# smithlabcode/walt

Measured on AMD Instinct MI355X. Metric: mapped reads/sec (100 bp single-end, hg19-scale index, -m 6 -b 5000), higher is better.
Workload: dtype u32

## Files before the change

### walt_amd/csrc/device_common.h

```cpp
#ifndef WALT_AMD_DEVICE_COMMON_H_
#define WALT_AMD_DEVICE_COMMON_H_

#include <hip/hip_runtime.h>

#include <initializer_list>
#include <mutex>
#include <string>
#include <type_traits>
#include <vector>

#include "../../include/walt_amd.h"
#include "batch_host.h"
#include "host_common.h"
#include "index_core.h"

#define WALT_HIP(expr)                                                                       \
  do {                                                                                       \
    hipError_t e_ = (expr);                                                                  \
    if (e_ != hipSuccess)                                                                    \
      return walt::fail(WALT_EHIP, std::string(#expr) + ": " + hipGetErrorString(e_));       \
  } while (0)

#define WALT_HIP_FORKED(expr)                                                                \
  do {                                                                                       \
    hipError_t e_ = (expr);                                                                  \
    if (e_ != hipSuccess) {                                                                  \
      unwind();                                                                              \
      return walt::fail(WALT_EHIP, std::string(#expr) + ": " + hipGetErrorString(e_));       \
    }                                                                                        \
  } while (0)

struct walt_options {
  int se_pipe = 1;
  long long se_heavy_chunk = 0;
  int se_stage_blocks = 0;
  int se_verify_blocks = 0;
  int se_stagger = 0;
  int se_lit_ablate = 0;
  int se_lit_side = 1;
  int se_lit_staged = 0;
  long long se_defer_min = -1;
  int se_stage_occ = 0;
  int se_carry = 1;
  int se_heavy_mono = 0;
  long long grid = 0;
  int pe_mode = 0;
  long long pe_chunk = 0;
  long long pe_rounds = 0;
  long long pe_stage_cap = 0;
  int pe_small_heaps = 0;
  int pe_serial = 0;
  int pe_push_wide = 0;
  long long pe_defer_min = -1;
  int pe_lit_fuse = 1;
  int pe_roomy = -1;
  int pile_rows = 0;
  long long pile_extract_blocks = 0;
};

struct walt_index {
  int device = 0;
  int n_cu = 256;
  walt_options opt;
  walt::IndexHead head;
  std::vector<uint32_t> start_index;
  walt::IndexView view;
  std::vector<void*> allocs;
// ... 267 lines not shown
```

### walt_amd/csrc/device_index.hip

```cpp
#include <fcntl.h>
#include <stdio.h>
#include <stdlib.h>
#include <string.h>
#include <time.h>
#include <unistd.h>

#include <algorithm>
#include <atomic>
#include <cstring>
#include <thread>

#include <hip/hip_runtime.h>
#include <rocprim/rocprim.hpp>

#include <stddef.h>

#include "device_common.h"

namespace walt {


__global__ void k_pack_genome(const uint8_t* __restrict__ bytes, uint32_t len, uint32_t ga,
                              uint32_t* __restrict__ g2, uint32_t nwords, uint32_t* __restrict__ err) {
  uint32_t w = blockIdx.x * blockDim.x + threadIdx.x;
// ... 988 lines not shown
}
const char* walt_index_chrom_name(const walt_index* idx, uint32_t i) {
  return idx && i < idx->head.names.size() ? idx->head.names[i].c_str() : "";
}
uint64_t walt_index_genome_len(const walt_index* idx) { return idx ? idx->head.genome_len : 0; }
uint64_t walt_index_device_bytes(const walt_index* idx) { return idx ? idx->device_bytes : 0; }
int walt_index_dir_bits(const walt_index* idx) { return idx ? (int)idx->view.dir_bits : -1; }
uint64_t walt_index_bad_buckets(const walt_index* idx, int strand) {
  return idx && strand >= 0 && strand < 4 ? idx->bad_buckets[strand] : 0;
}
namespace {
struct OptionName {
  const char* name;
  int kind;
  size_t offset;
  long long lo, hi;
};
#define WALT_OPT_I(f, lo, hi) {#f, 0, offsetof(walt_options, f), lo, hi}
#define WALT_OPT_L(f, lo, hi) {#f, 1, offsetof(walt_options, f), lo, hi}
const OptionName kOptions[] = {
    WALT_OPT_I(se_pipe, 0, 1),        WALT_OPT_L(se_heavy_chunk, 0, 1ll << 28), WALT_OPT_I(se_lit_staged, 0, 1), WALT_OPT_I(se_stage_blocks, 0, 16), WALT_OPT_I(se_verify_blocks, 0, 16), WALT_OPT_I(se_stagger, 0, 1), WALT_OPT_I(se_lit_side, 0, 2), WALT_OPT_I(se_lit_ablate, 0, 7),
    WALT_OPT_L(se_defer_min, -1, 1ll << 30), WALT_OPT_I(se_stage_occ, 0, 4),   WALT_OPT_I(se_carry, 0, 1),
    WALT_OPT_I(se_heavy_mono, 0, 1),  WALT_OPT_L(grid, 0, 1ll << 20),           WALT_OPT_I(pe_mode, 0, 1),
    WALT_OPT_L(pe_chunk, 0, 1ll << 28), WALT_OPT_L(pe_rounds, 0, 4),            WALT_OPT_L(pe_stage_cap, 0, 1ll << 28),
    WALT_OPT_I(pe_small_heaps, 0, 1), WALT_OPT_I(pe_serial, 0, 1), WALT_OPT_I(pe_push_wide, 0, 1),              WALT_OPT_L(pe_defer_min, -1, 1ll << 30),
    WALT_OPT_I(pe_roomy, -1, 1),      WALT_OPT_I(pe_lit_fuse, 0, 1),
    WALT_OPT_I(pile_rows, 0, 1),      WALT_OPT_L(pile_extract_blocks, 0, 1ll << 16),
};
#undef WALT_OPT_I
#undef WALT_OPT_L
const OptionName* find_option(const char* name) {
  if (!name) return nullptr;
  for (const OptionName& o : kOptions)
    if (!strcmp(o.name, name)) return &o;
  return nullptr;
}
}

int walt_index_set_option(walt_index* idx, const char* name, long long value) {
  if (!idx) return fail(WALT_EINVAL, "null index");
  const OptionName* o = find_option(name);
  if (!o) return fail(WALT_EINVAL, std::string("walt_index_set_option: unknown option '") + (name ? name : "(null)") + "'");
  if (value < o->lo || value > o->hi)
    return fail(WALT_EINVAL, std::string("walt_index_set_option: ") + name + " = " + std::to_string(value) + " is outside [" +
                                 std::to_string(o->lo) + ", " + std::to_string(o->hi) + "]");
  char* base = reinterpret_cast<char*>(&idx->opt) + o->offset;
// ... 25 lines not shown
```

### walt_amd/csrc/map_se.hip

```cpp
#include <stdio.h>
#include <stdlib.h>
#include <string.h>

#include "map_common.h"
#include "map_items.h"

namespace walt {

static __global__ __launch_bounds__(kBlock) void k_ascii_to_2bit(const uint8_t* __restrict__ bases,
                                                                  const uint64_t* __restrict__ offsets, uint32_t n,
                                                                  uint32_t* __restrict__ codes2, uint64_t cap_bytes,
                                                                  uint32_t* __restrict__ err) {
  const uint64_t o0 = offsets[0], all = offsets[n] - o0, total = all < cap_bytes ? all : cap_bytes;
  if (all > cap_bytes && blockIdx.x == 0 && threadIdx.x == 0) atomicAdd(err + 1, 1u);
  const uint8_t* src = bases + o0;
  const uint32_t mis = (uint32_t)(reinterpret_cast<uintptr_t>(src) & 15);
  const uint64_t nwords = (total + 15) / 16;
  uint32_t bad_total = 0;
  for (uint64_t i = (uint64_t)blockIdx.x * blockDim.x + threadIdx.x; i < nwords;
       i += (uint64_t)gridDim.x * blockDim.x) {
    uint32_t qs[4] = {0, 0, 0, 0};
    const uint64_t b0 = 16 * i;
    if (mis == 0 && b0 + 16 <= total) {
      const uint4 q = *reinterpret_cast<const uint4*>(src + b0);
      qs[0] = q.x; qs[1] = q.y; qs[2] = q.z; qs[3] = q.w;
    } else {
      for (uint64_t k = b0; k < b0 + 16; ++k) {
        const uint32_t c = k < total ? src[k] : 0x41u;
// ... 1369 lines not shown
  ItemQueue q;
  q.items = hs.items; q.ctl = hs.ctl; q.cap = 2 * hs.hcap; q.ovf = err + 2;
  q.bigs = hs.giants; q.big_n = hs.ctl + 5; q.big_cap = hs.hcap / 8;
  if (DENSE && blockIdx.x == 0 && threadIdx.x == 0) items_overflow_check(q);
  uint32_t n_big = DENSE ? *q.big_n : 0u;
  n_big = n_big < q.big_cap ? n_big : q.big_cap;
  const uint32_t n_items = q.ctl[DENSE ? 0 : 1] + n_big;
  if (n_items == 0) return;
  __shared__ uint32_t s_start[kLdsChroms + 1];
  __shared__ uint32_t s_edge[DENSE ? kEdgeWords : 1];
  const bool fits = iv.n_chrom <= kLdsChroms;
  chrom_tab_stage(s_start, iv.start_index, chrom_tab_of(iv.n_chrom));
  if (DENSE && iv.edge_bits != nullptr)
    for (uint32_t i = threadIdx.x; i < kEdgeWords; i += blockDim.x) s_edge[i] = iv.edge_bits[i];
  __syncthreads();
  const uint32_t* const edge = (DENSE && iv.edge_bits != nullptr) ? s_edge : nullptr;
  SummarySink sink;
  sink.sums = hs.sums; sink.hcap = hs.hcap; sink.n_verified = 0; sink.b = b; sink.tail = 0; sink.in_region = 0;
  if (fits) item_stream<NW, DENSE, true, SummarySink, G>(iv, strand_base, q, n_items, s_start, sink, n_big, edge);
  else item_stream<NW, DENSE, false, SummarySink, G>(iv, strand_base, q, n_items, s_start, sink, n_big, edge);
  flush_counters({0u, sink.n_verified, 0u}, 0u, stats);
}

#ifndef WALT_LIT_OCC
#define WALT_LIT_OCC 5
#endif
template <int NW, bool LITERAL = true>
__global__ __launch_bounds__(kBlock, NW <= 8 ? WALT_LIT_OCC : 1) void k_map_se_literal(IndexView iv, const uint32_t* __restrict__ codes2,
                                                            const uint64_t* __restrict__ offsets,
                                                            uint32_t* __restrict__ err, uint32_t strand_base,
                                                            uint32_t max_mm,
                                                            uint32_t b, const uint32_t* __restrict__ mask_table,
                                                            BestMatch* __restrict__ out,
                                                            unsigned long long* __restrict__ stats,
                                                            uint32_t* __restrict__ defer_count,
                                                            uint32_t* __restrict__ defer_list,
                                                            uint32_t all_reads, const uint32_t* __restrict__ range = nullptr) {
  uint32_t n_entries = 0;
  if (range != nullptr) {
    const uint32_t lo_entry = range[0];
    n_entries = range[1] > lo_entry ? range[1] - lo_entry : 0u;
    if (n_entries == 0) return;
    defer_list += lo_entry;
  }
  __shared__ BlockShared sh;
  const uint32_t* si = block_prologue(sh, iv, mask_table, strand_base);
// ... 39 lines not shown
}
static SeGeometry se_geometry_for(uint32_t n, int nw, bool pipe, uint64_t chunk_hook) {
  SeGeometry g;
  const uint64_t share = ((uint64_t)n + (pipe ? 7 : 3)) / (pipe ? 8 : 4);
  g.hcap = (uint32_t)align_up(n <= 65536 ? (n ? n : 1) : (share > 65536 ? share : 65536), 64);
  if (chunk_hook > 0 && chunk_hook * 8 >= n) g.hcap = (uint32_t)align_up(chunk_hook, 64);
  const uint32_t k = (uint32_t)(((uint64_t)n + g.hcap - 1) / g.hcap);
  g.piped = pipe && k > 1;
  g.chunks = g.piped ? (k + 1u) & ~1u : k;
  g.slot_bytes = se_heavy_slot_bytes(g.hcap, nw);
  g.heavy_bytes = 16 + kHeavyCtlWords * 4 + (g.piped ? 2 : 1) * g.slot_bytes;
  return g;
}
static uint64_t se_heavy_bytes(uint32_t n, int nw) {
  const uint64_t a = se_geometry_for(n, nw, true, 0).heavy_bytes, c = se_geometry_for(n, nw, false, 0).heavy_bytes;
  return a > c ? a : c;
}
static SeGeometry se_geometry(uint32_t n, int nw, const walt_options& opt) {
  SeGeometry g = se_geometry_for(n, nw, opt.se_pipe != 0, opt.se_heavy_chunk > 0 ? (uint64_t)opt.se_heavy_chunk : 0);
  if (g.heavy_bytes > se_heavy_bytes(n, nw) || g.hcap > (1u << kStageJBits)) g = se_geometry_for(n, nw, opt.se_pipe != 0, 0);
  return g;
}
static uint64_t se_carry_bytes(uint32_t n) { return (uint64_t)kPat * se_stride(n) * 16; }

constexpr unsigned kLiteralGrid = 2048;

#if defined(WALT_DIAG)
static uint32_t g_ablate = 0;
static unsigned long long* g_stamps = nullptr;
static void debug_sync(const char* what, hipStream_t stream) {
  static const bool on = getenv("WALT_AMD_SYNC_DEBUG") != nullptr;
  if (!on) return;
  const hipError_t e = hipStreamSynchronize(stream);
  fprintf(stderr, "[walt_amd sync] %s: %s\n", what, hipGetErrorString(e));
}
#else
static void debug_sync(const char*, hipStream_t) {}
#endif

unsigned persistent_grid(const walt_index* idx) {
  return idx->opt.grid > 0 ? (unsigned)idx->opt.grid : (unsigned)idx->n_cu * 8u;
}

template <int NW>
static int launch_map_se(walt_index* idx, const IndexView& view, const uint32_t* codes2, const uint64_t* offsets, uint32_t* err,
                         uint32_t n, uint32_t strand_base, uint32_t max_mm, uint32_t b, BestMatch* out,
                         unsigned long long* stats, uint32_t* defer_count, uint32_t* defer_list, uint64_t stride,
                         uint32_t* heavy_area, uint4* carry_area, hipStream_t stream) {
  const walt_options& opt = idx->opt;
  const unsigned pg = persistent_grid(idx);
  const unsigned g1 = grid_for(n) < pg ? grid_for(n) : pg;
  uint32_t* heavy_count = defer_count + 24;
  uint32_t* heavy_list = defer_list + 2 * stride;
  const bool mono = opt.se_heavy_mono != 0;
  SeCarry carry;
  carry.st = (opt.se_carry && !mono) ? carry_area : nullptr;
  carry.neg = carry_area + stride;
  carry.stride = stride;
  idx->n_detail = 0;
  auto mark = [&](unsigned char kind) {
    if (!idx->profile || idx->n_detail >= walt_index::kDetailEvents) return;
    hipEvent_t& e = idx->ev_detail[idx->n_detail];
    if (!e && hipEventCreate(&e) != hipSuccess) return;
    if (hipEventRecord(e, stream) != hipSuccess) return;
    idx->ev_kind[idx->n_detail++] = kind;
  };
  mark(255);
#if defined(WALT_DIAG)
  const bool diag = g_ablate != 0 || g_stamps != nullptr;
  const char* sm = getenv("WALT_AMD_STAMPS");
  const int stamp_mode = sm ? atoi(sm) : 0;
// ... 21 lines not shown
  };
  uint32_t* const rng = heavy_area + kHeavyCtlWords - 8;
  if (mono) {
#if defined(WALT_DIAG)
    if (diag2)
      hipLaunchKernelGGL((k_map_se<NW, true, true>), dim3(g1), dim3(kBlock), 0, stream, view, codes2, offsets, err, n,
                         strand_base, max_mm, b, idx->d_mask_table, out, stats, defer_count, defer_list, heavy_count,
                         heavy_list, g_ablate, g_stamps, SeCarry());
    else
#endif
      hipLaunchKernelGGL((k_map_se<NW, false, true>), dim3(g1), dim3(kBlock), 0, stream, view, codes2, offsets, err, n,
                         strand_base, max_mm, b, idx->d_mask_table, out, stats, defer_count, defer_list, heavy_count,
                         heavy_list, 0u, nullptr, SeCarry());
  } else {
    const SeGeometry geo = se_geometry(n, NW, opt);
    const uint32_t hcap = geo.hcap;
    const bool piped = geo.piped && !diag;
    const uint32_t chunks = geo.chunks;
    HeavyStage hs;
    hs.ctl = heavy_area;
    hs.hcap = hcap;
    hs.even = piped ? 1u : 0u;
    const uint64_t slot_words = geo.slot_bytes / 4;
    auto use_slot = [&](uint32_t k, uint32_t*& lists) {
      lists = heavy_area + kHeavyCtlWords + k * slot_words;
      hs.st = reinterpret_cast<uint4*>(lists + (uint64_t)kPat * hcap);
      hs.rdq = hs.st + hcap;
      hs.sums = hs.rdq + (uint64_t)rd_quads<NW>() * hcap;
      hs.items = hs.sums + (uint64_t)(kPat + 1) * hcap;
      hs.giants = hs.items + (uint64_t)2 * hcap * item_quads<NW>();
    };
    hs.defer_min = opt.se_defer_min < 0 ? (uint32_t)kSmallRegion
                 : opt.se_defer_min == 0 ? 0xFFFFFFFFu
                 : (uint32_t)(opt.se_defer_min < (long long)kSmallRegion ? (long long)kSmallRegion : opt.se_defer_min);
    hs.lit_ablate = (uint32_t)opt.se_lit_ablate;
    uint32_t* const ctl0 = heavy_area;
    static const int vb_dense = [] {
      int nb = 0;
      if (hipOccupancyMaxActiveBlocksPerMultiprocessor(&nb, k_se_verify<NW, NW <= 10>, kBlock, 0) != hipSuccess || nb < 1) nb = 4;
      return nb;
    }();
    static const int vb_gather = [] {
      int nb = 0;
      if (hipOccupancyMaxActiveBlocksPerMultiprocessor(&nb, k_se_verify<NW, false>, kBlock, 0) != hipSuccess || nb < 1) nb = 2;
      return nb;
    }();
    const unsigned vg_dense = (unsigned)vb_dense * (unsigned)idx->n_cu, vg_gather = (unsigned)vb_gather * (unsigned)idx->n_cu;
    const bool lit_staged = opt.se_lit_staged != 0 && !diag;
    lit_side = !lit_staged && opt.se_lit_side != 0 && !diag && n <= kDeferMask;
    uint32_t* const ctl2 = ctl0 + 64 * kPat;
    uint32_t* const rng_side = ctl2 + 32;
    static_assert(8 * kPat * kLitChunks >= 34, "the side launch's control words fit the literal rounds' area");
    if (lit_side && !idx->se_side) {
      int lo_pri = 0, hi_pri = 0;
      WALT_HIP(hipDeviceGetStreamPriorityRange(&lo_pri, &hi_pri));
      WALT_HIP(create_stream_set(&idx->se_side, &lo_pri, {&idx->se_fork, &idx->se_join}));
    }
    if (piped && !idx->se_pipe)
      WALT_HIP(create_stream_set(&idx->se_pipe, nullptr, {&idx->se_pipe_ev[0], &idx->se_pipe_ev[1], &idx->se_pipe_ev[2]}));
    const bool lit_early = lit_side && opt.se_lit_side >= 2;
    if (lit_early) {
      hipLaunchKernelGGL(k_lit_snapshot, dim3(1), dim3(64), 0, stream, defer_count, ctl2, rng_side);
      WALT_HIP(hipEventRecord(idx->se_fork, stream));
      WALT_HIP(hipStreamWaitEvent(idx->se_side, idx->se_fork, 0));
      forked = true;
      launch_bin_deferred(ctl2, defer_list, defer_list + stride, idx->se_side);
      const unsigned g_lit = grid_for(n) < kLiteralGrid ? grid_for(n) : kLiteralGrid;
      hipLaunchKernelGGL(k_map_se_literal<NW>, dim3(g_lit), dim3(kBlock), 0, idx->se_side, view, codes2, offsets, err,
                         strand_base, max_mm, b, idx->d_mask_table, out, stats, ctl2, defer_list + stride, 0u);
// ... 39 lines not shown
            WALT_HIP_FORKED(hipEventRecord(idx->se_fork, cs));
            WALT_HIP_FORKED(hipStreamWaitEvent(idx->se_side, idx->se_fork, 0));
            launch_bin_deferred(ctl3, defer_list, defer_list + stride, idx->se_side, ctl3 + 1);
            const unsigned g_lit = grid_for(n) < kLiteralGrid ? grid_for(n) : kLiteralGrid;
            hipLaunchKernelGGL(k_map_se_literal<NW>, dim3(g_lit), dim3(kBlock), 0, idx->se_side, view, codes2, offsets, err,
                               strand_base, max_mm, b, idx->d_mask_table, out, stats, defer_count, defer_list + stride, 0u, ctl3 + 24);
            WALT_HIP_FORKED(hipEventRecord(idx->se_join, idx->se_side));
          }
          if (lit_side && !lit_early && c_side == (piped ? 1u : 0u)) {
            if (piped) WALT_HIP_FORKED(hipStreamWaitEvent(cs, idx->se_pipe_ev[1], 0));
            hipLaunchKernelGGL(k_lit_snapshot, dim3(1), dim3(64), 0, cs, defer_count, ctl2, rng_side);
            WALT_HIP_FORKED(hipEventRecord(idx->se_fork, cs));
            WALT_HIP_FORKED(hipStreamWaitEvent(idx->se_side, idx->se_fork, 0));
            forked = true;
            launch_bin_deferred(ctl2, defer_list, defer_list + stride, idx->se_side);
            const unsigned g_lit = grid_for(n) < kLiteralGrid ? grid_for(n) : kLiteralGrid;
            hipLaunchKernelGGL(k_map_se_literal<NW>, dim3(g_lit), dim3(kBlock), 0, idx->se_side, view, codes2, offsets, err,
                               strand_base, max_mm, b, idx->d_mask_table, out, stats, ctl2, defer_list + stride, 0u);
            WALT_HIP_FORKED(hipEventRecord(idx->se_join, idx->se_side));
          }
        }
        if constexpr (NW <= 10 && long_seed_nw<NW>())
          hipLaunchKernelGGL((k_se_tail_narrow<NW>), dim3(pg), dim3(kBlock), 0, cs, view, strand_base, hs, b);
        if constexpr (NW <= 10) {
          hipLaunchKernelGGL((k_se_verify<NW, true>), dim3(vgd), dim3(kBlock), 0, cs, view, strand_base, stats, hs, b, err);
        }
        hipLaunchKernelGGL((k_se_verify<NW, false>), dim3(vg_gather), dim3(kBlock), 0, cs, view, strand_base, stats, hs, b, err);
        if (marks) mark(lit ? 3 : 2);
      }
      return WALT_OK;
    };
    for (uint32_t c = 0; c < chunks; ++c) {
      const bool odd = piped && (c & 1u);
      forked = forked || odd;
      uint32_t* lists = nullptr;
      use_slot(odd ? 1u : 0u, lists);
      hs.first = c * hcap;
      hs.chunk = c;
      if (piped && lit_side && !lit_early && c == 2) WALT_HIP_FORKED(hipStreamWaitEvent(stream, idx->se_fork, 0));
      const int rc_chunk = run_chunk(odd ? idx->se_pipe : stream, ctl0 + 8 * kPat * c, lists, false, heavy_count, heavy_list, carry, !odd, c);
      if (rc_chunk) return rc_chunk;
    }
    if (piped) {
      WALT_HIP_FORKED(hipEventRecord(idx->se_pipe_ev[2], idx->se_pipe));
      WALT_HIP_FORKED(hipStreamWaitEvent(stream, idx->se_pipe_ev[2], 0));
    }
    if (lit_staged) {
      hs.even = 0;
// ... 51 lines not shown
    WALT_HIP(hipMemset(g_stamps, 0, 16 * sizeof(unsigned long long)));
  }
  return WALT_OK;
}
#endif

static int se_check_len(uint32_t max_read_len, int& nw) {
  nw = nw_for_len(max_read_len);
  if (!nw) return fail(WALT_EINVAL, "read length above 1024 is not supported (reference line limit is 1000, util.hpp:43)");
  if (max_read_len > kMaxReadLen)
    return fail(WALT_EINVAL, "reads longer than " + std::to_string(kMaxReadLen) + " bases are outside the tables of seed pattern " +
                                 std::to_string(kPat) + " (seedpattern.hpp)");
  return WALT_OK;
}

struct SeWorkspace {
  uint32_t* err;
  unsigned long long* shards;
  uint32_t* defer_count;
  uint32_t* defer_list;
  uint32_t* codes2;
  uint32_t* heavy_area;
  uint4* carry_area;
  uint64_t stride;
  uint64_t end;
};
static SeWorkspace se_workspace(void* d_workspace, uint32_t n, uint32_t max_read_len, int nw) {
  SeWorkspace w;
  w.stride = se_stride(n);
  w.err = reinterpret_cast<uint32_t*>(d_workspace);
  w.shards = reinterpret_cast<unsigned long long*>(w.err + 64);
  w.defer_count = w.err + 32;
  w.defer_list = w.err + 64 + kStatShardBytes / 4;
  w.codes2 = w.defer_list + 3 * w.stride;
  w.heavy_area = reinterpret_cast<uint32_t*>(
      align_up(reinterpret_cast<uint64_t>(w.codes2 + codes2_words((uint64_t)n * max_read_len)), 16));
  w.carry_area = reinterpret_cast<uint4*>(align_up(reinterpret_cast<uint64_t>(w.heavy_area) + se_heavy_bytes(n, nw), 16));
  w.end = reinterpret_cast<uint64_t>(w.carry_area) + se_carry_bytes(n);
  return w;
}

static int se_map_pass(walt_index* idx, const IndexView& view, const SeWorkspace& w, const uint64_t* offsets, uint32_t n,
                       int nw, uint32_t sb, uint32_t max_mm, uint32_t b, BestMatch* out, hipStream_t stream) {
  return dispatch_nw(nw, [&](auto NW) {
    return launch_map_se<decltype(NW)::value>(idx, view, w.codes2, offsets, w.err, n, sb, max_mm, b, out, w.shards, w.defer_count,
                                              w.defer_list, w.stride, w.heavy_area, w.carry_area, stream);
  });
}

struct SeCall {
  std::unique_lock<std::mutex> busy;
  int nw = 0;
  SeWorkspace w;
  IndexView view;
  const uint64_t* offsets = nullptr;
};
static int se_begin(walt_index* idx, bool rp, bool locked, const void* d_bases, const void* d_offsets, uint32_t n,
                    uint32_t max_read_len, void* d_workspace, size_t workspace_bytes, hipStream_t stream, SeCall& c) {
  const std::string entry = rp ? "walt_map_se_rpbat_batch" : "walt_map_se_batch";
  if (n > kDeferMask + 1) return fail(WALT_EINVAL, "more than 2^28 reads in one batch (the reference's -N limit is 10^8, walt.cpp:236-239)");
  if (!locked)
    if (const int rc_busy = take_busy(c.busy, idx->se_busy, entry.c_str(), "single-end")) return rc_busy;
#if defined(WALT_DIAG)
  if (const int rc_diag = se_diag_setup()) return rc_diag;
#endif
  if (const int rc_len = se_check_len(max_read_len, c.nw)) return rc_len;
  const size_t need = rp ? walt_se_rpbat_workspace_bytes(n, max_read_len) : walt_se_workspace_bytes(n, max_read_len);
  if (workspace_bytes < need)
    return fail(WALT_EINVAL, entry + "_device: the workspace holds " + std::to_string(workspace_bytes) + " bytes, the call needs " +
                                 std::to_string(need) + (rp ? " (walt_se_rpbat_workspace_bytes)" : " (walt_se_workspace_bytes)"));
  WALT_HIP(hipSetDevice(idx->device));
  c.w = se_workspace(d_workspace, n, max_read_len, c.nw);
  WALT_HIP(hipMemsetAsync(c.w.err, 0, 64 * sizeof(uint32_t) + kStatShardBytes, stream));
  WALT_HIP(hipMemsetAsync(c.w.heavy_area, 0, kHeavyCtlWords * sizeof(uint32_t), stream));
  c.offsets = reinterpret_cast<const uint64_t*>(d_offsets);
  if (idx->profile) WALT_HIP(hipEventRecord(idx->ev[0], stream));
  c.view = idx->view;
  c.view.batch_max_len = max_read_len;
  c.view.batch_cap_bytes = (uint64_t)n * max_read_len;
  launch_ascii_to_2bit(reinterpret_cast<const uint8_t*>(d_bases), c.offsets, n, c.w.codes2, c.view.batch_cap_bytes, c.w.err, stream);
  if (idx->profile) WALT_HIP(hipEventRecord(idx->ev[1], stream));
  return WALT_OK;
}

int map_se_device(walt_index* idx, const void* d_bases, const void* d_offsets, uint32_t n, uint32_t max_read_len,
                  int ag, uint32_t max_mm, uint32_t b, void* d_out, void* d_stats, void* d_workspace,
                  size_t workspace_bytes, hipStream_t stream, bool locked) {
  if (!idx) return fail(WALT_EINVAL, "null index");
  const unsigned need = ag ? WALT_STRANDS_GA : WALT_STRANDS_CT;
  if ((idx->strand_mask & need) != need)
    return fail(WALT_EINVAL, ag ? "index opened without the _GA10/_GA11 strands" : "index opened without the _CT00/_CT01 strands");
  if (n == 0) return WALT_OK;
  SeCall c;
  if (const int rc = se_begin(idx, false, locked, d_bases, d_offsets, n, max_read_len, d_workspace, workspace_bytes, stream, c)) return rc;
  const int rc = se_map_pass(idx, c.view, c.w, c.offsets, n, c.nw, ag ? 2u : 0u, max_mm, b, reinterpret_cast<BestMatch*>(d_out), stream);
  if (rc) return rc;
  launch_reduce_stats(c.w.shards, reinterpret_cast<unsigned long long*>(d_stats), stream);
// ... 41 lines not shown
    return fail(WALT_EINVAL, "walt_map_se_rpbat_batch: the index was opened without the strands " + missing +
                                 " (random PBAT maps under both conversions: open it with WALT_STRANDS_ALL)");
  }
  if (n == 0) return WALT_OK;
  if (!d_out || !d_conv || !d_stats || !d_workspace || (reinterpret_cast<uintptr_t>(d_out) & 15) ||
      (reinterpret_cast<uintptr_t>(d_workspace) & 15))
    return fail(WALT_EINVAL, "walt_map_se_rpbat_batch_device: bad argument (null pointer, or d_out / d_workspace not 16-byte aligned)");
  SeCall c;
  int rc = se_begin(idx, true, locked, d_bases, d_offsets, n, max_read_len, d_workspace, workspace_bytes, stream, c);
  if (rc) return rc;
  const SeWorkspace& w = c.w;
  uint4* const ga = reinterpret_cast<uint4*>(reinterpret_cast<uint8_t*>(d_workspace) + se_rpbat_ga_offset(n, max_read_len));
  unsigned long long* stats = reinterpret_cast<unsigned long long*>(d_stats);
  rc = se_map_pass(idx, c.view, w, c.offsets, n, c.nw, 0u, max_mm, b, reinterpret_cast<BestMatch*>(d_out), stream);
  if (rc) return rc;
  auto unwind = [&]() {
    if (idx->se_pipe) (void)hipStreamSynchronize(idx->se_pipe);
    if (idx->se_side) (void)hipStreamSynchronize(idx->se_side);
  };
  launch_reduce_stats(w.shards, stats, stream);
  WALT_HIP_FORKED(hipGetLastError());
  WALT_HIP_FORKED(hipMemsetAsync(w.err + 3, 0, 61 * sizeof(uint32_t), stream));
  WALT_HIP_FORKED(hipMemsetAsync(w.heavy_area, 0, kHeavyCtlWords * sizeof(uint32_t), stream));
  rc = se_map_pass(idx, c.view, w, c.offsets, n, c.nw, 2u, max_mm, b, reinterpret_cast<BestMatch*>(ga), stream);
  if (rc) {
    unwind();
    return rc;
  }
  const unsigned gm = grid_for(n) < (unsigned)idx->n_cu * 4u ? grid_for(n) : (unsigned)idx->n_cu * 4u;
  hipLaunchKernelGGL(k_se_rpbat_merge, dim3(gm), dim3(kBlock), 0, stream, reinterpret_cast<uint4*>(d_out), ga,
                     reinterpret_cast<uint8_t*>(d_conv), n);
  hipLaunchKernelGGL(k_reduce_stats<1>, dim3(1), dim3(kStatShards), 0, stream, w.shards, stats);
  if (idx->profile) {
    WALT_HIP_FORKED(hipEventRecord(idx->ev[2], stream));
    idx->ev_valid = true;
  }
  WALT_HIP_FORKED(hipGetLastError());
  return WALT_OK;
}

int check_read_errors(const void* d_workspace, hipStream_t stream) {
  uint32_t herr[3] = {0, 0, 0};
  WALT_HIP(hipMemcpyAsync(herr, d_workspace, sizeof(herr), hipMemcpyDeviceToHost, stream));
  WALT_HIP(hipStreamSynchronize(stream));
  if (herr[2]) return fail(WALT_EHIP, "internal: a work-item queue of the heavy pass overflowed (" + std::to_string(herr[2]) + " items dropped); results are incomplete");
  if (herr[1]) return fail(WALT_EINVAL, "reads longer than max_read_len, or more bases than n x max_read_len (" + std::to_string(herr[1]) + " refusals)");
// ... 61 lines not shown
  for (int i = 1; i < idx->n_detail; ++i) {
    float ms = 0.f;
    WALT_HIP(hipEventElapsedTime(&ms, idx->ev_detail[i - 1], idx->ev_detail[i]));
    if (idx->ev_kind[i] < 4) out4[idx->ev_kind[i]] += ms;
  }
  return WALT_OK;
}

int walt_profile_last(walt_index* idx, float* pack_ms, float* map_ms) {
  if (!idx || !idx->profile || !idx->ev_valid) return fail(WALT_EINVAL, "no profiled call recorded");
  WALT_HIP(hipEventSynchronize(idx->ev[2]));
  float a = 0, b = 0;
  WALT_HIP(hipEventElapsedTime(&a, idx->ev[0], idx->ev[1]));
  WALT_HIP(hipEventElapsedTime(&b, idx->ev[1], idx->ev[2]));
  if (pack_ms) *pack_ms = a;
  if (map_ms) *map_ms = b;
  return WALT_OK;
}

size_t walt_se_workspace_bytes(uint32_t n, uint32_t max_read_len) {
  int nw = nw_for_len(max_read_len);
  if (!nw) nw = 64;
  return 64 * sizeof(uint32_t) + kStatShardBytes + 3 * se_stride(n) * sizeof(uint32_t) +
         codes2_words((uint64_t)n * max_read_len) * sizeof(uint32_t) + 16 + se_heavy_bytes(n, nw) + 16 + se_carry_bytes(n);
}

int walt_map_se_batch_device(walt_index* idx, const void* d_bases, const void* d_offsets, uint32_t n,
                             uint32_t max_read_len, int ag_wildcard, uint32_t max_mismatches, uint32_t b,
                             void* d_out, void* d_stats, void* d_workspace, size_t workspace_bytes, void* stream) {
  return map_se_device(idx, d_bases, d_offsets, n, max_read_len, ag_wildcard, max_mismatches, b, d_out, d_stats,
                       d_workspace, workspace_bytes, reinterpret_cast<hipStream_t>(stream), false);
}

static int se_host_call(walt_index* idx, const char* bases, const uint64_t* offsets, uint32_t n, int ag, uint32_t max_mm,
                        uint32_t b, walt_best_match* out, uint8_t* conv, bool rp, walt_batch_stats* stats) {
  const std::string entry = rp ? "walt_map_se_rpbat_batch" : "walt_map_se_batch";
  if (!idx || !offsets || (!bases && n && offsets[n] > 0) || (!out && n) || (rp && !conv && n)) return fail(WALT_EINVAL, entry + ": bad argument");
  if (stats) memset(stats, 0, sizeof(*stats));
  if (n == 0) return WALT_OK;
  uint32_t max_len = 0;
  if (const char* bad = scan_offsets(offsets, n, &max_len)) return fail(WALT_EINVAL, bad);
  std::unique_lock<std::mutex> busy;
  if (const int rc_busy = take_busy(busy, idx->se_busy, entry.c_str(), "single-end")) return rc_busy;
  WALT_HIP(hipSetDevice(idx->device));
  const size_t ws_bytes = rp ? walt_se_rpbat_workspace_bytes(n, max_len) : walt_se_workspace_bytes(n, max_len);
  HostUpload up{idx};
  void *d_bases = nullptr, *d_off = nullptr;
// ... 39 lines not shown
```

Baseline: 1.348 billion.

## Group heavy verify items sharing a candidate range so one wavefront verifies several reads

Adds a hash-bucket sort (count, scan, scatter) of dense-verify items keyed by strand and record start. A wavefront-level cut pass then packs items with identical candidate ranges into units of up to four reads. A new shared verify kernel loads each genome window once and checks it against every read in the unit, replacing the per-item dense verify by default. This removes redundant window loads, at the cost of extra sort and cut kernels, more workspace, an added memset and more register pressure from per-read accumulators.

Result: faster. 1.458 billion (median of 6 runs) (+8.2%).

```diff
diff --git a/walt_amd/csrc/device_common.h b/walt_amd/csrc/device_common.h
--- a/walt_amd/csrc/device_common.h
+++ b/walt_amd/csrc/device_common.h
@@ -43,6 +43,9 @@
   int se_stage_occ = 0;
   int se_carry = 1;
   int se_heavy_mono = 0;
+  int se_verify_share = 1;
+  int se_share_r = 0;
+  long long se_share_cap = 0;
   long long grid = 0;
   int pe_mode = 0;
   long long pe_chunk = 0;
diff --git a/walt_amd/csrc/device_index.hip b/walt_amd/csrc/device_index.hip
--- a/walt_amd/csrc/device_index.hip
+++ b/walt_amd/csrc/device_index.hip
@@ -1034,6 +1034,7 @@
     WALT_OPT_I(se_pipe, 0, 1),        WALT_OPT_L(se_heavy_chunk, 0, 1ll << 28), WALT_OPT_I(se_lit_staged, 0, 1), WALT_OPT_I(se_stage_blocks, 0, 16), WALT_OPT_I(se_verify_blocks, 0, 16), WALT_OPT_I(se_stagger, 0, 1), WALT_OPT_I(se_lit_side, 0, 2), WALT_OPT_I(se_lit_ablate, 0, 7),
     WALT_OPT_L(se_defer_min, -1, 1ll << 30), WALT_OPT_I(se_stage_occ, 0, 4),   WALT_OPT_I(se_carry, 0, 1),
     WALT_OPT_I(se_heavy_mono, 0, 1),  WALT_OPT_L(grid, 0, 1ll << 20),           WALT_OPT_I(pe_mode, 0, 1),
+    WALT_OPT_I(se_verify_share, 0, 2), WALT_OPT_I(se_share_r, 0, 64),           WALT_OPT_L(se_share_cap, 0, 1ll << 30),
     WALT_OPT_L(pe_chunk, 0, 1ll << 28), WALT_OPT_L(pe_rounds, 0, 4),            WALT_OPT_L(pe_stage_cap, 0, 1ll << 28),
     WALT_OPT_I(pe_small_heaps, 0, 1), WALT_OPT_I(pe_serial, 0, 1), WALT_OPT_I(pe_push_wide, 0, 1),              WALT_OPT_L(pe_defer_min, -1, 1ll << 30),
     WALT_OPT_I(pe_roomy, -1, 1),      WALT_OPT_I(pe_lit_fuse, 0, 1),
diff --git a/walt_amd/csrc/group_core.h b/walt_amd/csrc/group_core.h
--- /dev/null
+++ b/walt_amd/csrc/group_core.h
@@ -0,0 +1,74 @@
+#ifndef WALT_AMD_GROUP_CORE_H_
+#define WALT_AMD_GROUP_CORE_H_
+
+#include <stdint.h>
+
+#if !defined(WALT_HD)
+#if defined(__HIPCC__)
+#define WALT_HD __host__ __device__ __forceinline__
+#else
+#define WALT_HD inline
+#endif
+#endif
+
+namespace walt {
+
+constexpr uint32_t kGroupBucketBits = 16;
+constexpr uint32_t kGroupBuckets = 1u << kGroupBucketBits;
+constexpr uint32_t kGroupSlice = 64;
+constexpr uint32_t kGroupRMax = kGroupSlice;
+
+WALT_HD uint64_t group_key(uint32_t id, uint32_t rec0) { return ((uint64_t)(id >> 31) << 32) | rec0; }
+
+WALT_HD uint32_t group_bucket(uint64_t key) {
+  return (uint32_t)((key * 0x9E3779B97F4A7C15ull) >> (64 - kGroupBucketBits));
+}
+
+WALT_HD bool group_joins(uint64_t key, uint32_t size, uint32_t tail, uint64_t lead_key, uint32_t lead_size, uint32_t lead_tail) {
+  return tail == 0 && lead_tail == 0 && key == lead_key && size == lead_size;
+}
+
+struct GroupPlace {
+  uint32_t pos;
+  uint32_t unit_first;
+  uint32_t unit_n;
+  bool leads;
+};
+WALT_HD uint32_t group_popc(unsigned long long m) {
+#if defined(__HIP_DEVICE_COMPILE__)
+  return (uint32_t)__popcll(m);
+#else
+  return (uint32_t)__builtin_popcountll(m);
+#endif
+}
+WALT_HD GroupPlace group_place(unsigned long long m, uint32_t lane, uint32_t placed, uint32_t r) {
+  const uint32_t rank = group_popc(m & ((1ull << lane) - 1ull)), n = group_popc(m);
+  const uint32_t first = rank / r * r;
+  GroupPlace p;
+  p.pos = placed + rank;
+  p.unit_first = placed + first;
+  p.unit_n = n - first < r ? n - first : r;
+  p.leads = rank == first;
+  return p;
+}
+
+#if !defined(__HIP_DEVICE_COMPILE__)
+inline void group_cut_slice(const uint64_t* key, const uint32_t* size, const uint32_t* tail, uint32_t n, uint32_t r, GroupPlace* place) {
+  unsigned long long rem = n >= 64 ? ~0ull : (1ull << n) - 1ull;
+  uint32_t placed = 0;
+  while (rem) {
+    const uint32_t ld = (uint32_t)__builtin_ctzll(rem);
+    unsigned long long m = 0;
+    for (uint32_t t = 0; t < n; ++t)
+      if (t == ld || group_joins(key[t], size[t], tail[t], key[ld], size[ld], tail[ld])) m |= 1ull << t;
+    m &= rem;
+    for (uint32_t t = 0; t < n; ++t)
+      if ((m >> t) & 1ull) place[t] = group_place(m, t, placed, r);
+    placed += group_popc(m);
+    rem &= ~m;
+  }
+}
+#endif
+
+}
+#endif
diff --git a/walt_amd/csrc/map_se.hip b/walt_amd/csrc/map_se.hip
--- a/walt_amd/csrc/map_se.hip
+++ b/walt_amd/csrc/map_se.hip
@@ -4,6 +4,7 @@
 
 #include "map_common.h"
 #include "map_items.h"
+#include "group_core.h"
 
 namespace walt {
 
@@ -1419,6 +1420,363 @@
   flush_counters({0u, sink.n_verified, 0u}, 0u, stats);
 }
 
+template <int NW>
+constexpr bool share_nw() { return NW <= 8 && !(kPat != 3 && long_seed_nw<NW>()); }
+constexpr int kShareR = 4;
+constexpr uint32_t kShareRounds = 8 * kPat;
+struct SeShare {
+  uint32_t* count;
+  uint32_t* cursor;
+  uint32_t* order;
+  uint2* units;
+  uint32_t* ctl;
+  unsigned long long* recs;
+  uint32_t cap;
+  uint32_t r;
+};
+__device__ __forceinline__ void share_counts(const HeavyStage& hs, uint32_t& n_big, uint32_t& n_all) {
+  const uint32_t g = hs.ctl[5], d = hs.ctl[0];
+  n_big = g < hs.hcap / 8 ? g : hs.hcap / 8;
+  n_all = n_big + (d < 2 * hs.hcap ? d : 2 * hs.hcap);
+}
+template <int NW>
+__device__ __forceinline__ const uint4* share_item(const HeavyStage& hs, uint32_t i, uint32_t n_big) {
+  constexpr uint32_t Q = item_quads<NW>();
+  return i < n_big ? hs.giants + (uint64_t)Q * i : hs.items + (uint64_t)Q * (i - n_big);
+}
+__device__ __forceinline__ unsigned long long wave_sum_u64(unsigned long long v) {
+#pragma unroll
+  for (int off = 32; off > 0; off >>= 1) v += __shfl_xor(v, off);
+  return v;
+}
+
+template <int NW, bool SCATTER>
+__global__ __launch_bounds__(kBlock) void k_se_share_bin(HeavyStage hs, SeShare sh) {
+  uint32_t n_big, n_all;
+  share_counts(hs, n_big, n_all);
+  const uint32_t n_grp = n_all < sh.cap ? n_all : sh.cap;
+  unsigned long long beyond = 0;
+  for (uint32_t i = blockIdx.x * blockDim.x + threadIdx.x; i < (SCATTER ? n_grp : n_all); i += gridDim.x * blockDim.x) {
+    const uint4 h = load_global(share_item<NW>(hs, i, n_big));
+    if (i < n_grp) {
+      const uint32_t bk = group_bucket(group_key(h.x, h.w));
+      if constexpr (SCATTER) {
+        const uint32_t at = atomicAdd(&sh.cursor[bk], 1u);
+        if (at < sh.cap) sh.order[at] = i;
+      } else {
+        atomicAdd(&sh.count[bk], 1u);
+      }
+    } else {
+      beyond += h.z;
+    }
+  }
+  if constexpr (!SCATTER) {
+    if (n_all > n_grp) {
+      beyond = wave_sum_u64(beyond);
+      if ((threadIdx.x & 63) == 0 && beyond) {
+        atomicAdd(&sh.recs[0], beyond);
+        atomicAdd(&sh.recs[1], beyond);
+      }
+    }
+  }
+}
+
+constexpr uint32_t kShareScanThreads = 1024;
+__global__ __launch_bounds__(kShareScanThreads) void k_se_share_scan(SeShare sh) {
+  constexpr uint32_t per = kGroupBuckets / kShareScanThreads;
+  __shared__ uint32_t part[kShareScanThreads];
+  const uint32_t t = threadIdx.x;
+  uint32_t s = 0;
+  for (uint32_t k = 0; k < per; ++k) s += sh.count[t * per + k];
+  part[t] = s;
+  __syncthreads();
+  for (uint32_t off = 1; off < kShareScanThreads; off <<= 1) {
+    const uint32_t v = t >= off ? part[t - off] : 0u;
+    __syncthreads();
+    part[t] += v;
+    __syncthreads();
+  }
+  uint32_t run = part[t] - s;
+  for (uint32_t k = 0; k < per; ++k) {
+    sh.cursor[t * per + k] = run;
+    run += sh.count[t * per + k];
+    sh.count[t * per + k] = 0u;
+  }
+}
+
+template <int NW>
+__global__ __launch_bounds__(kBlock) void k_se_share_cut(HeavyStage hs, SeShare sh) {
+  uint32_t n_big, n_all;
+  share_counts(hs, n_big, n_all);
+  const uint32_t lane = threadIdx.x & 63;
+  const uint32_t n_waves = (gridDim.x * blockDim.x) >> 6, wave = (blockIdx.x * blockDim.x + threadIdx.x) >> 6;
+  const uint32_t r = sh.r ? sh.r : 1u;
+  unsigned long long rec_items = 0, rec_units = 0;
+  uint32_t rode = 0;
+  const uint32_t end = n_all < sh.cap ? n_all : sh.cap;
+  for (uint32_t s = wave * kGroupSlice; s < end; s += n_waves * kGroupSlice) {
+    const uint32_t p = s + lane;
+    const bool valid = p < end;
+    uint32_t item = sh.order[valid ? p : s];
+    item = item < n_all ? item : 0u;
+    const uint4* it = share_item<NW>(hs, item, n_big);
+    const uint4 h0 = load_global(it), h1 = load_global(it + 1);
+    const uint64_t key = group_key(h0.x, h0.w);
+    const uint32_t size = h0.z, tail = h1.z;
+    unsigned long long rem = __ballot(valid);
+    uint32_t placed = 0;
+    GroupPlace mine = {0u, 0u, 1u, true};
+    while (rem) {
+      const int ld = (int)__ffsll((long long)rem) - 1;
+      const uint64_t lkey = group_key(bcast(h0.x, ld), bcast(h0.w, ld));
+      const bool join = (int)lane == ld || group_joins(key, size, tail, lkey, bcast(size, ld), bcast(tail, ld));
+      const unsigned long long m = __ballot(join) & rem;
+      if ((m >> lane) & 1ull) mine = group_place(m, lane, placed, r);
+      placed += (uint32_t)__popcll(m);
+      rem &= ~m;
+    }
+    if (valid) sh.order[s + mine.pos] = item;
+    const bool leads = valid && mine.leads, big = size > kBigFirst;
+    const unsigned long long mb = __ballot(leads && big), mr = __ballot(leads && !big);
+    uint32_t base_b = 0, base_r = 0;
+    if (lane == 0) {
+      if (mb) base_b = atomicAdd(&sh.ctl[0], (uint32_t)__popcll(mb));
+      if (mr) base_r = atomicAdd(&sh.ctl[1], (uint32_t)__popcll(mr));
+    }
+    base_b = bcast(base_b, 0);
+    base_r = bcast(base_r, 0);
+    if (leads) {
+      const unsigned long long below = (1ull << lane) - 1ull;
+      const uint32_t k = big ? base_b + (uint32_t)__popcll(mb & below) : base_r + (uint32_t)__popcll(mr & below);
+      if (k < sh.cap) sh.units[big ? k : sh.cap - 1u - k] = make_uint2(mine.unit_n == 1u ? item : s + mine.unit_first, mine.unit_n);
+    }
+    rec_items += valid ? size : 0u;
+    rec_units += leads ? size : 0u;
+    rode += (valid && !mine.leads) ? 1u : 0u;
+  }
+  rec_items = wave_sum_u64(rec_items);
+  rec_units = wave_sum_u64(rec_units);
+  rode = wave_sum_u32(rode);
+  if (lane == 0) {
+    if (rec_items) atomicAdd(&sh.recs[0], rec_items);
+    if (rec_units) atomicAdd(&sh.recs[1], rec_units);
+    if (rode) atomicAdd(&hs.ctl[7], rode);
+  }
+}
+
+template <int NW, int R>
+__global__ __launch_bounds__(kBlock, NW > 7 ? 4 : 5) void k_se_verify_shared(
+    IndexView iv, uint32_t strand_base, unsigned long long* __restrict__ stats, HeavyStage hs, SeShare sh, uint32_t b,
+    uint32_t* __restrict__ err) {
+  static_assert(share_nw<NW>() && item_quads<NW>() <= 8 && R >= 1 && R <= 8, "a unit's headers are fetched by one wavefront load");
+  constexpr uint32_t Q = item_quads<NW>();
+  {
+    ItemQueue q;
+    q.items = hs.items; q.ctl = hs.ctl; q.cap = 2 * hs.hcap; q.ovf = err + 2;
+    if (blockIdx.x == 0 && threadIdx.x == 0) items_overflow_check(q);
+  }
+  uint32_t n_big, n_all;
+  share_counts(hs, n_big, n_all);
+  if (n_all == 0) return;
+  const uint32_t n_grp = n_all < sh.cap ? n_all : sh.cap;
+  uint32_t nbu = sh.ctl[0], nru = sh.ctl[1];
+  nbu = nbu < sh.cap ? nbu : sh.cap;
+  nru = nru < sh.cap - nbu ? nru : sh.cap - nbu;
+  const uint32_t nu = nbu + nru, n_units = nu + (n_all - n_grp);
+  __shared__ uint32_t s_start[kLdsChroms + 1];
+  __shared__ uint32_t s_edge[kEdgeWords];
+  const bool fits = iv.n_chrom <= kLdsChroms;
+  chrom_tab_stage(s_start, iv.start_index, chrom_tab_of(iv.n_chrom));
+  const bool has_edge = iv.edge_bits != nullptr;
+  if (has_edge)
+    for (uint32_t i = threadIdx.x; i < kEdgeWords; i += blockDim.x) s_edge[i] = iv.edge_bits[i];
+  __syncthreads();
+  const uint32_t n_chrom = iv.n_chrom, top_step = top_step_of(n_chrom);
+  const uint32_t lane = threadIdx.x & 63;
+  const uint32_t n_waves = (gridDim.x * blockDim.x) >> 6, wave = (blockIdx.x * blockDim.x + threadIdx.x) >> 6;
+  uint32_t n_verified = 0;
+  if (wave < n_units) {
+  uint32_t* const cursor = &sh.ctl[2];
+  const bool many = n_units >= 32 * n_waves;
+  uint32_t batch = many ? n_units / (4 * n_waves) : 2u;
+  batch = batch > kVerifyBatchMax ? kVerifyBatchMax : batch;
+  const uint32_t first_batch = many ? batch : (uint32_t)((3ull * n_units + 4ull * n_waves - 1) / (4ull * n_waves));
+  const uint32_t dealt = n_waves * first_batch;
+  auto grab = [&]() {
+    uint32_t v = 0;
+    if (lane == 0) v = dealt + atomicAdd(cursor, batch);
+    return v;
+  };
+  uint32_t b0 = wave, t = 0, stride = n_waves, cur_batch = first_batch, nb_v = 0;
+  uint32_t deal = 0;
+  if (cur_batch == 1 && dealt < n_units) {
+    nb_v = grab();
+    deal = 1u;
+  }
+  auto advance = [&]() __attribute__((always_inline)) -> uint32_t {
+    if (deal & 2u) return 0xFFFFFFFFu;
+    uint32_t ni;
+    if (t + 1 < cur_batch) {
+      ++t;
+      ni = b0 + t * stride;
+    } else {
+      b0 = (deal & 1u) ? bcast(nb_v, 0) : 0xFFFFFFFFu;
+      deal = 0u;
+      t = 0;
+      ni = b0;
+      cur_batch = batch;
+      stride = 1;
+    }
+    if (ni >= n_units) {
+      deal = 2u;
+      return 0xFFFFFFFFu;
+    }
+    if (t + 1 == cur_batch && dealt < n_units) {
+      nb_v = grab();
+      deal = 1u;
+    }
+    return ni;
+  };
+  auto unit_entry = [&](uint32_t i) __attribute__((always_inline)) -> uint2 {
+    const bool on = i < nu;
+    const uint64_t at = !on ? 0ull : (i < nbu ? (uint64_t)i : (uint64_t)sh.cap - 1u - (i - nbu));
+    uint2 e = load_global(sh.units + at);
+    if (!on) e = make_uint2(i < n_units ? sh.cap + (i - nu) : 0u, i < n_units ? 1u : 0u);
+    e.x = (uint32_t)__builtin_amdgcn_readfirstlane((int)e.x);
+    e.y = (uint32_t)__builtin_amdgcn_readfirstlane((int)e.y);
+    e.y = e.y < (uint32_t)R ? e.y : (uint32_t)R;
+    return e;
+  };
+  const uint32_t rr = lane >> 3, qq = lane & 7u;
+  auto headers = [&](const uint2& e) __attribute__((always_inline)) -> uint4 {
+    uint32_t item = e.x;
+    if (e.y > 1u) {
+      const uint32_t p = e.x + (rr < e.y ? rr : 0u);
+      item = sh.order[p < sh.cap ? p : 0u];
+    }
+    item = item < n_all ? item : 0u;
+    return load_global(share_item<NW>(hs, item, n_big) + ((rr < e.y && qq < Q) ? qq : 0u));
+  };
+  auto chrom_bounds_of = [&](uint32_t pos, uint32_t& c_lo, uint32_t& c_hi) {
+    if (has_edge && !((s_edge[pos >> (kEdgeBlockShift + 5)] >> ((pos >> kEdgeBlockShift) & 31u)) & 1u)) {
+      c_lo = 0; c_hi = 0xFFFFFFFFu;
+      return;
+    }
+    if (fits) {
+      const uint32_t chr = chrom_id_steps(s_start, n_chrom, top_step, pos);
+      c_lo = s_start[chr]; c_hi = s_start[chr + 1];
+    } else {
+      walt::chrom_bounds(s_start, iv.start_index, chrom_tab_of(n_chrom), pos, c_lo, c_hi);
+    }
+  };
+  struct Buf { uint4 a, c, e; };
+  const uint4 zero = make_uint4(0, 0, 0, 0);
+  Buf bx, by;
+  bx.a = bx.c = bx.e = by.a = by.c = by.e = zero;
+  auto issue = [&](uint32_t fi, uint32_t r0, uint32_t sz, uint32_t base, Buf& y) {
+    fi = (uint32_t)__builtin_amdgcn_readfirstlane((int)fi);
+    r0 = (uint32_t)__builtin_amdgcn_readfirstlane((int)r0);
+    sz = (uint32_t)__builtin_amdgcn_readfirstlane((int)sz);
+    const StrandView& sv = iv.s[strand_base + fi];
+    const uint32_t k = base + lane;
+    const uint64_t rec = (uint64_t)r0 + (k < sz ? k : sz - 1);
+    const uint4* rp = reinterpret_cast<const uint4*>(sv.win) + 2 * rec;
+    y.a = load_global(rp);
+    y.c = load_global(rp + 1);
+    if constexpr (NW > 7) y.e = load_global(reinterpret_cast<const uint4*>(sv.win2) + rec);
+  };
+  uint2 ue = unit_entry(wave);
+  uint4 hv = headers(ue);
+  uint32_t i1 = advance();
+  uint2 ue1 = unit_entry(i1);
+  uint4 hv1 = headers(ue1);
+  uint32_t i2 = advance();
+  uint2 ue2 = unit_entry(i2);
+  LaneBest acc[R];
+  uint32_t strand = 0, size = 1, rec0 = 0, base = 0;
+  auto begin = [&]() {
+    strand = bcast(hv.x, 0) >> 31; size = bcast(hv.z, 0); rec0 = bcast(hv.w, 0);
+    size = size ? size : 1u;
+#pragma unroll
+    for (int r = 0; r < R; ++r) acc[r] = {0xFFFFFFFFu, 0u, 0u, 0u, 0u, 0u};
+    base = 0;
+  };
+  bool done = false;
+  auto step = [&](Buf& x, Buf& y) {
+    const bool last = base + 64 >= size;
+    const bool hn = i1 != 0xFFFFFFFFu;
+    uint32_t n_fi = strand, n_rec0 = rec0, n_size = size;
+    const uint32_t n_base = last ? 0u : base + 64;
+    if (last && hn) {
+      n_fi = bcast(hv1.x, 0) >> 31; n_size = bcast(hv1.z, 0); n_rec0 = bcast(hv1.w, 0);
+      n_size = n_size ? n_size : 1u;
+    }
+    issue(n_fi, n_rec0, n_size, n_base, y);
+    const uint32_t k = base + lane;
+    const uint32_t pos = x.a.x;
+    uint32_t c_lo, c_hi;
+    chrom_bounds_of(pos, c_lo, c_hi);
+    uint32_t wv[NW + 1];
+    const uint32_t first[11] = {x.a.y, x.a.z, x.a.w, x.c.x, x.c.y, x.c.z, x.c.w, NW > 7 ? x.e.x : 0u, NW > 7 ? x.e.y : 0u,
+                                NW > 7 ? x.e.z : 0u, NW > 7 ? x.e.w : 0u};
+#pragma unroll
+    for (int w = 0; w <= NW; ++w) wv[w] = first[w];
+#pragma unroll
+    for (int r = 0; r < R; ++r) {
+      if ((uint32_t)r < ue.y) {
+        const uint32_t len = bcast(hv.x, 8 * r + 1), seed_i = bcast(hv.y, 8 * r + 1);
+        uint32_t rd[NW], mk[NW];
+#pragma unroll
+        for (int w = 0; w < NW; ++w) {
+          const int a = 8 + w, c = 8 + NW + w;
+          const uint32_t va = (a & 3) == 0 ? hv.x : (a & 3) == 1 ? hv.y : (a & 3) == 2 ? hv.z : hv.w;
+          const uint32_t vc = (c & 3) == 0 ? hv.x : (c & 3) == 1 ? hv.y : (c & 3) == 2 ? hv.z : hv.w;
+          rd[w] = bcast(va, 8 * r + (a >> 2));
+          mk[w] = bcast(vc, 8 * r + (c >> 2));
+        }
+        const uint32_t g = pos - seed_i;
+        const bool ok = k < size && (pos - c_lo >= seed_i) && (g + len < c_hi);
+        const uint32_t m = count_mismatch_regs<NW>(wv, 2 * (kWinLead - seed_i), rd, mk);
+        n_verified += ok ? 1u : 0u;
+        lane_best_add(acc[r], k, ok ? g : 0u, ok ? m : 0xFFFFFFFFu);
+      }
+    }
+    if (last) {
+#pragma unroll
+      for (int r = 0; r < R; ++r) {
+        if ((uint32_t)r < ue.y) {
+          const uint32_t id = bcast(hv.x, 8 * r), seed_i = bcast(hv.y, 8 * r + 1), tail = bcast(hv.z, 8 * r + 1);
+          uint4 res = lane_best_reduce(acc[r]);
+          if (tail && size > b) res = make_uint4(0xFFFFFFFFu, 0u, 0u, 0u);
+          if (lane == 0) hs.sums[(uint64_t)((id >> 31) ? 1u + seed_i : 0u) * hs.hcap + (id & 0x7FFFFFFFu)] = res;
+        }
+      }
+      if (hn) {
+        ue = ue1; hv = hv1;
+        i1 = i2; ue1 = ue2;
+        hv1 = headers(ue1);
+        i2 = advance();
+        ue2 = unit_entry(i2);
+        begin();
+      } else {
+        done = true;
+      }
+    } else {
+      base += 64;
+    }
+  };
+  begin();
+  issue(strand, rec0, size, 0u, bx);
+  for (;;) {
+    step(bx, by);
+    if (done) break;
+    step(by, bx);
+    if (done) break;
+  }
+  }
+  flush_counters({0u, n_verified, 0u}, 0u, stats);
+}
+
 #ifndef WALT_LIT_OCC
 #define WALT_LIT_OCC 5
 #endif
@@ -1504,6 +1862,28 @@
   return g;
 }
 static uint64_t se_carry_bytes(uint32_t n) { return (uint64_t)kPat * se_stride(n) * 16; }
+constexpr uint64_t kShareCtlWords = 4 * kShareRounds;
+constexpr uint64_t kShareZeroBytes = 2ull * kGroupBuckets * 4 + kShareCtlWords * 4 + kShareRounds * 2 * 8;
+constexpr uint64_t kShareCursorBytes = 2ull * kGroupBuckets * 4;
+static uint64_t se_share_slot_bytes(uint64_t cap_items) { return align_up((cap_items & ~1ull) * 12, 16); }
+static uint64_t se_share_big_bytes(uint32_t n, int nw) {
+  if (nw > 8) return 0;
+  uint64_t most = 0;
+  for (int pipe = 0; pipe < 2; ++pipe) {
+    const SeGeometry g = se_geometry_for(n, nw, pipe != 0, 0);
+    const uint64_t v = (g.piped ? 2 : 1) * se_share_slot_bytes(2ull * g.hcap + g.hcap / 8);
+    most = v > most ? v : most;
+  }
+  return most;
+}
+static uint64_t se_share_bytes(uint32_t n, int nw) { return 32 + se_share_big_bytes(n, nw) + kShareCursorBytes + kShareZeroBytes; }
+static uint32_t se_share_cap_for(const SeGeometry& g, uint64_t slot_bytes, long long hook) {
+  const uint64_t full = 2ull * g.hcap + g.hcap / 8;
+  uint64_t cap = slot_bytes / 12;
+  cap = (cap < full ? cap : full) & ~1ull;
+  if (hook > 0 && (uint64_t)hook < cap) cap = (uint64_t)hook;
+  return (uint32_t)cap;
+}
 
 constexpr unsigned kLiteralGrid = 2048;
 
@@ -1524,11 +1904,24 @@
   return idx->opt.grid > 0 ? (unsigned)idx->opt.grid : (unsigned)idx->n_cu * 8u;
 }
 
+struct SeShareArea {
+  uint8_t* big = nullptr;
+  uint64_t big_bytes = 0;
+  uint32_t* zero = nullptr;
+};
+
+template <class K>
+static int occupancy_blocks(K kernel) {
+  int nb = 0;
+  if (hipOccupancyMaxActiveBlocksPerMultiprocessor(&nb, kernel, kBlock, 0) != hipSuccess || nb < 1) nb = 4;
+  return nb;
+}
+
 template <int NW>
 static int launch_map_se(walt_index* idx, const IndexView& view, const uint32_t* codes2, const uint64_t* offsets, uint32_t* err,
                          uint32_t n, uint32_t strand_base, uint32_t max_mm, uint32_t b, BestMatch* out,
                          unsigned long long* stats, uint32_t* defer_count, uint32_t* defer_list, uint64_t stride,
-                         uint32_t* heavy_area, uint4* carry_area, hipStream_t stream) {
+                         uint32_t* heavy_area, uint4* carry_area, const SeShareArea& share_area, hipStream_t stream) {
   const walt_options& opt = idx->opt;
   const unsigned pg = persistent_grid(idx);
   const unsigned g1 = grid_for(n) < pg ? grid_for(n) : pg;
@@ -1596,6 +1989,12 @@
     hs.hcap = hcap;
     hs.even = piped ? 1u : 0u;
     const uint64_t slot_words = geo.slot_bytes / 4;
+    SeShare sh = {};
+    const uint64_t share_slot = (share_area.big_bytes / (geo.piped ? 2 : 1)) & ~15ull;
+    const uint32_t share_alloc = se_share_cap_for(geo, share_slot, 0);
+    sh.cap = se_share_cap_for(geo, share_slot, opt.se_share_cap);
+    int share_mode = (share_nw<NW>() && !diag && share_area.zero != nullptr && sh.cap > 0) ? opt.se_verify_share : 0;
+    sh.r = (share_mode == 2 && opt.se_share_r > 0) ? (uint32_t)opt.se_share_r : (uint32_t)kShareR;
     auto use_slot = [&](uint32_t k, uint32_t*& lists) {
       lists = heavy_area + kHeavyCtlWords + k * slot_words;
       hs.st = reinterpret_cast<uint4*>(lists + (uint64_t)kPat * hcap);
@@ -1603,6 +2002,12 @@
       hs.sums = hs.rdq + (uint64_t)rd_quads<NW>() * hcap;
       hs.items = hs.sums + (uint64_t)(kPat + 1) * hcap;
       hs.giants = hs.items + (uint64_t)2 * hcap * item_quads<NW>();
+      if (share_mode) {
+        sh.count = share_area.zero + k * kGroupBuckets;
+        sh.cursor = share_area.zero - (2 - k) * kGroupBuckets;
+        sh.order = reinterpret_cast<uint32_t*>(share_area.big + k * share_slot);
+        sh.units = reinterpret_cast<uint2*>(sh.order + share_alloc);
+      }
     };
     hs.defer_min = opt.se_defer_min < 0 ? (uint32_t)kSmallRegion
                  : opt.se_defer_min == 0 ? 0xFFFFFFFFu
@@ -1619,6 +2024,14 @@
       if (hipOccupancyMaxActiveBlocksPerMultiprocessor(&nb, k_se_verify<NW, false>, kBlock, 0) != hipSuccess || nb < 1) nb = 2;
       return nb;
     }();
+    auto share_blocks = []() -> int {
+      if constexpr (share_nw<NW>()) {
+        static const int nb = occupancy_blocks(k_se_verify_shared<NW, kShareR>);
+        return nb;
+      } else {
+        return 4;
+      }
+    };
     const unsigned vg_dense = (unsigned)vb_dense * (unsigned)idx->n_cu, vg_gather = (unsigned)vb_gather * (unsigned)idx->n_cu;
     const bool lit_staged = opt.se_lit_staged != 0 && !diag;
     lit_side = !lit_staged && opt.se_lit_side != 0 && !diag && n <= kDeferMask;
@@ -1704,8 +2117,26 @@
         }
         if constexpr (NW <= 10 && long_seed_nw<NW>())
           hipLaunchKernelGGL((k_se_tail_narrow<NW>), dim3(pg), dim3(kBlock), 0, cs, view, strand_base, hs, b);
+        bool shared_done = false;
+        if constexpr (share_nw<NW>()) {
+          if (share_mode && !lit && c_side < 8u) {
+            sh.ctl = share_area.zero + 2 * kGroupBuckets + 4 * (c_side * kPat + round);
+            sh.recs = reinterpret_cast<unsigned long long*>(share_area.zero + 2 * kGroupBuckets + kShareCtlWords) + 2 * (c_side * kPat + round);
+            const unsigned gs = (unsigned)idx->n_cu;
+            hipLaunchKernelGGL((k_se_share_bin<NW, false>), dim3(gs), dim3(kBlock), 0, cs, hs, sh);
+            hipLaunchKernelGGL(k_se_share_scan, dim3(1), dim3(kShareScanThreads), 0, cs, sh);
+            hipLaunchKernelGGL((k_se_share_bin<NW, true>), dim3(gs), dim3(kBlock), 0, cs, hs, sh);
+            hipLaunchKernelGGL((k_se_share_cut<NW>), dim3(gs), dim3(kBlock), 0, cs, hs, sh);
+            if (share_mode == 1) {
+              const unsigned vgs = (opt.se_verify_blocks > 0 ? (unsigned)opt.se_verify_blocks : (unsigned)share_blocks()) * (unsigned)idx->n_cu;
+              hipLaunchKernelGGL((k_se_verify_shared<NW, kShareR>), dim3(vgs), dim3(kBlock), 0, cs, view, strand_base, stats, hs, sh, b, err);
+              shared_done = true;
+            }
+          }
+        }
         if constexpr (NW <= 10) {
-          hipLaunchKernelGGL((k_se_verify<NW, true>), dim3(vgd), dim3(kBlock), 0, cs, view, strand_base, stats, hs, b, err);
+          if (!shared_done)
+            hipLaunchKernelGGL((k_se_verify<NW, true>), dim3(vgd), dim3(kBlock), 0, cs, view, strand_base, stats, hs, b, err);
         }
         hipLaunchKernelGGL((k_se_verify<NW, false>), dim3(vg_gather), dim3(kBlock), 0, cs, view, strand_base, stats, hs, b, err);
         if (marks) mark(lit ? 3 : 2);
@@ -1803,6 +2234,7 @@
   uint32_t* codes2;
   uint32_t* heavy_area;
   uint4* carry_area;
+  SeShareArea share;
   uint64_t stride;
   uint64_t end;
 };
@@ -1817,7 +2249,10 @@
   w.heavy_area = reinterpret_cast<uint32_t*>(
       align_up(reinterpret_cast<uint64_t>(w.codes2 + codes2_words((uint64_t)n * max_read_len)), 16));
   w.carry_area = reinterpret_cast<uint4*>(align_up(reinterpret_cast<uint64_t>(w.heavy_area) + se_heavy_bytes(n, nw), 16));
-  w.end = reinterpret_cast<uint64_t>(w.carry_area) + se_carry_bytes(n);
+  w.share.big = reinterpret_cast<uint8_t*>(align_up(reinterpret_cast<uint64_t>(w.carry_area) + se_carry_bytes(n), 16));
+  w.share.big_bytes = se_share_big_bytes(n, nw);
+  w.end = (reinterpret_cast<uint64_t>(d_workspace) + walt_se_workspace_bytes(n, max_read_len)) & ~15ull;
+  w.share.zero = reinterpret_cast<uint32_t*>(w.end - kShareZeroBytes);
   return w;
 }
 
@@ -1825,7 +2260,7 @@
                        int nw, uint32_t sb, uint32_t max_mm, uint32_t b, BestMatch* out, hipStream_t stream) {
   return dispatch_nw(nw, [&](auto NW) {
     return launch_map_se<decltype(NW)::value>(idx, view, w.codes2, offsets, w.err, n, sb, max_mm, b, out, w.shards, w.defer_count,
-                                              w.defer_list, w.stride, w.heavy_area, w.carry_area, stream);
+                                              w.defer_list, w.stride, w.heavy_area, w.carry_area, w.share, stream);
   });
 }
 
@@ -1854,6 +2289,7 @@
   c.w = se_workspace(d_workspace, n, max_read_len, c.nw);
   WALT_HIP(hipMemsetAsync(c.w.err, 0, 64 * sizeof(uint32_t) + kStatShardBytes, stream));
   WALT_HIP(hipMemsetAsync(c.w.heavy_area, 0, kHeavyCtlWords * sizeof(uint32_t), stream));
+  if (idx->opt.se_verify_share) WALT_HIP(hipMemsetAsync(c.w.share.zero, 0, kShareZeroBytes, stream));
   c.offsets = reinterpret_cast<const uint64_t*>(d_offsets);
   if (idx->profile) WALT_HIP(hipEventRecord(idx->ev[0], stream));
   c.view = idx->view;
@@ -1941,6 +2377,7 @@
   WALT_HIP_FORKED(hipGetLastError());
   WALT_HIP_FORKED(hipMemsetAsync(w.err + 3, 0, 61 * sizeof(uint32_t), stream));
   WALT_HIP_FORKED(hipMemsetAsync(w.heavy_area, 0, kHeavyCtlWords * sizeof(uint32_t), stream));
+  if (idx->opt.se_verify_share) WALT_HIP_FORKED(hipMemsetAsync(w.share.zero, 0, kShareZeroBytes, stream));
   rc = se_map_pass(idx, c.view, w, c.offsets, n, c.nw, 2u, max_mm, b, reinterpret_cast<BestMatch*>(ga), stream);
   if (rc) {
     unwind();
@@ -2048,7 +2485,8 @@
   int nw = nw_for_len(max_read_len);
   if (!nw) nw = 64;
   return 64 * sizeof(uint32_t) + kStatShardBytes + 3 * se_stride(n) * sizeof(uint32_t) +
-         codes2_words((uint64_t)n * max_read_len) * sizeof(uint32_t) + 16 + se_heavy_bytes(n, nw) + 16 + se_carry_bytes(n);
+         codes2_words((uint64_t)n * max_read_len) * sizeof(uint32_t) + 16 + se_heavy_bytes(n, nw) + 16 + se_carry_bytes(n) +
+         se_share_bytes(n, nw);
 }
 
 int walt_map_se_batch_device(walt_index* idx, const void* d_bases, const void* d_offsets, uint32_t n,
```
